# nantiferov/karpenter-sigs

Hardware: AMD Instinct MI355X
Metric: pods/sec in Scheduler.Solve @50k pods x 400 types (higher is better)
Workload: dtype int64; 1 GPU; C2: 50000 resource-only pods x 400 fake.InstanceTypes, 1 NodeClaimTemplate, no limits, empty topology (BenchmarkScheduling shape); pods=50000, instance_types=400, parallelism=replicas1, new_nodeclaims=122

## Files before the change

### karpenter-sigs_amd/csrc/ks_capi.cpp

```cpp
#include <hip/hip_runtime_api.h>

#include <algorithm>
#include <chrono>
#include <cstring>
#include <memory>
#include <mutex>
#include <string>
#include <vector>

#include "../../include/karpenter_amd.h"
#include "ks_archive.h"
#include "ks_feas.h"
#include "ks_feas_host.h"
#include "ks_host.h"
#include "ks_runtime.h"
#include "ks_sort_probe.h"

using namespace ks;

static thread_local std::string g_err;
namespace ks {
void set_last_error(const std::string& m) { g_err = m; }

static thread_local std::vector<Route>* g_routes = nullptr;
// ... 1092 lines not shown
  long long nfail = 0, nshared = 0, nverr = 0;
  for (char x : h.injectFailed) nfail += x ? 1 : 0;
  for (int32_t f : h.tab.pod_flags) {
    nshared += (f & PF_VSHARED) ? 1 : 0;
    nverr += (f & PF_VOLERR) ? 1 : 0;
  }
  kv("volAny", d.volAny); kv("volDrivers", d.VD); kv("volPvcs", d.NVU); kv("volLogCap", d.vLogCap);
  kv("volSharedPods", nshared); kv("volErrorPods", nverr); kv("injectFailed", nfail);
  kv("volStaticMounts", (long long)(h.tab.pod_vsbeg.empty() ? 0 : h.tab.pod_vsbeg.back()));
  o += "," + topo_inspect_json(h);
  std::vector<int32_t> frontBeg, frontPos;
  pareto_fronts(d, h.tab.tpl_it_beg, h.tab.tpl_its, h.tab.it_alloc, frontBeg, frontPos);
  o += ",\"runFuse\":" + std::to_string(run_fuse_build()) + ",\"sortLeaf\":" + std::to_string(sort_leaf_build()) +
       ",\"closedShift\":" + std::to_string(closed_shift_build()) + ",\"tplMasks\":" + std::to_string(tpl_masks_build()) +
       ",\"logRuns\":" + std::to_string(log_runs_build()) + ",\"sortRegs\":" + std::to_string(sort_regs_build()) +
       ",\"sortRegsN64\":" + std::to_string(sort_regs_n64_build()) + ",\"queuePacked\":" + std::to_string(queue_packed_build()) + ",\"paretoFronts\":[";
  for (int t = 0; t < d.NTPL; t++) {
    o += t ? ",[" : "[";
    for (int i = frontBeg[(size_t)t]; i < frontBeg[(size_t)t + 1]; i++)
      o += (i > frontBeg[(size_t)t] ? "," : "") + std::to_string(frontPos[(size_t)i]);
    o += "]";
  }
  o += "]";
  o += ",\"plans\":{";
  const size_t budgets[] = {160 * 1024 - 256, 6000, 9000, 14000, 24000, 40000};
  long long fnr = 0;
  for (int32_t f : h.tab.st_flags) fnr += (f & SF_HAS_KEYS) ? 1 : 0;
  KsDims pd = d;
  pd.fnOn = node_rows_on(d, (size_t)fnr);
  auto plan_json = [&](size_t budget, int wide) {
    Plan pl = make_plan(pd, budget, false, wide, (int)frontPos.size());
// ... 377 lines not shown
    ksjson::quote(o, r->errors[i].second);
  }
  o += "},\"stats\":{";
  static const char* names[] = {"nclaims", "ncommits", "hostnameCounter", "error", "pops", "algBytes",
                                "sorts", "sortsWithDescent", "claimFull", "claimQuickFail", "windows",
                                "cycPop", "cycNodes", "cycSort", "cycQuick", "cycFull", "cycCommit", "cycTemplates",
                                "cycTotal", "cycNodeCommit", "cycFullRs", "cycFullThr", "cycFullMasks", "cycFullApply",
                                "runs", "runPods", "sortsExact", "fineTopoPop", "fineState", "fineRefill",
                                "fineWindowTests", "fineWindowBlocks", "fineRecord", "fineNodeCommit", "fineWindowTopo",
                                "runCross", "runCrossStops", "runCrossLost", "sortsClosed", "tplMemoHits",
                                "cycSortFast", "cycSortExact", "cycSortClosed", "sortsLe12", "sortsLt50",
                                "cycRunCap", "cycCross", "cycBulk", "cycLog", "cycTplDerive", "cycTplStore",
                                "cycTplMax", "runCapFront", "runCapFull", "runCrossClosed", "runMoves",
                                "cycSortExactLe12", "cycSortExactLt50", "cycSortExactGe50", "closedShiftDiff",
                                "tplMaskFills", "tplMaskHits", "runRecs", "sortsRegs", "sortRegsBail", "sortRegsOver",
                                "cycTplCand", "cycTplFeas", "cycTplFilter", "cycTplThr", "cycLogLoad", "cycLogStore"};
  static_assert(sizeof(names) / sizeof(names[0]) == CT_NCOUNTERS, "one name per counter");
  for (int i = 0; i < CT_NCOUNTERS; i++) o += std::string(i ? "," : "") + "\"" + names[i] + "\":" + std::to_string(r->counters[i]);
  if (!r->routes.empty()) {
    std::string last = routes_json({r->routes.back()});
    o += ",\"route\":" + last.substr(1, last.size() - 3) + ",\"launches\":" + routes_json(r->routes) + "}";
  }
  o += ",\"plan\":{\"wide\":" + std::to_string(r->planWide) + ",\"KO\":" + std::to_string(r->plan.KO) +
       ",\"KL\":" + std::to_string(r->plan.KL) + ",\"talloc\":" + std::to_string(r->plan.talloc) +
       ",\"lds\":" + std::to_string(r->plan.lds) + "}";
  o += "}}";
  *json_out = strdup(o.c_str());
  return KS_OK;
  API_CATCH
}

// ... 304 lines not shown
```

### karpenter-sigs_amd/csrc/ks_problem.h

```cpp
#pragma once
#include <stdint.h>

#include "ks_reqset.h"

#if defined(__HIP_DEVICE_COMPILE__)
#define KS_G __attribute__((address_space(1)))
#define KS_L __attribute__((address_space(3)))
#define KS_C __attribute__((address_space(4)))
#else
#define KS_G
#define KS_L
#define KS_C
#endif

namespace ks {

constexpr int kMaxR = 16;
constexpr int kProbeMaxN = 1024;
constexpr int kMaxTpl = 64;
constexpr int kWave = 64;

enum PodStatus : int32_t { ST_PENDING = 0, ST_SCHEDULED = 1, ST_FAILED = 2 };
enum FailCode : uint32_t {
  FC_NONE = 0,
// ... 255 lines not shown
  CT_STEP,
  CT_RUN_CAP_FRONT = CT_STEP + 12,
  CT_RUN_CAP_FULL,
  CT_RUN_CROSS_CLOSED,
  CT_RUN_MOVES,
  CT_CYC_EXACT_BY_N,
  CT_CLOSED_SHIFT_DIFF = CT_CYC_EXACT_BY_N + 3,
  CT_TPL_MASK_FILLS,
  CT_TPL_MASK_HITS,
  CT_RUN_RECS,
  CT_SORT_REGS,
  CT_SORT_REGS_BAIL,
  CT_SORT_REGS_OVER,
  CT_CYC_SPLIT,
  CT_CYC_SPLIT_END = CT_CYC_SPLIT + 6,
  CT_NCOUNTERS = CT_CYC_SPLIT_END
};
enum SplitSub { YS_TPL_CAND = 0, YS_TPL_FEAS, YS_TPL_FILTER, YS_TPL_THR, YS_LOG_LOAD, YS_LOG_STORE };

enum StepSub {
  SS_SORT_FAST = 0,
  SS_SORT_EXACT,
  SS_SORT_CLOSED,
  SS_SORTS_LE12,
  SS_SORTS_LT50,
  SS_RUN_CAP,
  SS_CROSS,
  SS_BULK,
  SS_LOG,
  SS_TPL_DERIVE,
  SS_TPL_STORE,
  SS_TPL_MAX,
};
// ... 4 lines not shown
```

### karpenter-sigs_amd/csrc/ks_queue.hip

```cpp
#include <hip/hip_runtime.h>

#ifndef KS_QUEUE_PACKED
#define KS_QUEUE_PACKED 0
#endif

#include <hipcub/hipcub.hpp>

#include "ks_problem.h"

namespace ks {

__global__ void k_qkeys(const int64_t* sortkey, int comp, int64_t minv, const int32_t* perm, uint64_t* keys,
                        int32_t* vals, int n, int first) {
  const int i = blockIdx.x * blockDim.x + threadIdx.x;
  if (i >= n) return;
  const int p = first ? i : perm[i];
  keys[i] = (uint64_t)(sortkey[(int64_t)p * 4 + comp] - minv);
  vals[i] = p;
}

struct QPack {
  int64_t minv[4];
  int32_t shift[4];
  int32_t bits[4];
// ... 216 lines not shown
```

### karpenter-sigs_amd/csrc/ks_runtime.h

```cpp
#pragma once
#include <atomic>
#include <hip/hip_runtime_api.h>

#include <string>
#include <vector>

#include "../../include/karpenter_amd.h"
#include "ks_host.h"
#include "ks_tplmask.h"

namespace ks {
hipError_t launch_solve(const KsDev& D, const KsWork* works_dev, int nrep, const Plan& pl, int32_t* qorder,
                        uint64_t* skeys, int32_t* svals, void* stemp, size_t stempBytes, hipStream_t st,
                        hipEvent_t mid, const int32_t* fixed_order = nullptr, hipEvent_t* feas = nullptr,
                        int32_t* run_len = nullptr, uint64_t* run_words = nullptr, hipEvent_t post = nullptr);
hipError_t launch_sims(const KsDev& D, const KsWork* works_dev, int nsims, const Plan& pl, hipStream_t st);
hipError_t launch_sims_topo(const KsDev& D, const KsWork* w, int n, const Plan& pl, hipStream_t st);
void launch_feasibility(const KsDev& D, hipStream_t st);
void launch_feasibility_nodes(const KsDev& D, hipStream_t st);
bool sims_mw_supported(const KsDev& D, const Plan& pl);
hipError_t launch_sims_split(const KsDev& D, const KsWork* works_dev, int nsims, int nmw, const Plan& pl, hipStream_t st,
                             hipStream_t st2, hipEvent_t fork, hipEvent_t join);
int run_fuse_build();
int sort_leaf_build();
int closed_shift_build();
int tpl_masks_build();
int log_runs_build();
int sort_regs_build();
int sort_regs_n64_build();
int queue_packed_build();
hipError_t claim_sort_probe(int32_t* keys, int32_t* order, int n, int mode, int pos, int R, const int32_t* ctpl,
                            const int64_t* chead, int32_t* ptpl, int64_t* phead, int32_t* how, hipStream_t st);
Plan make_plan(const KsDims& d, size_t budget, bool sim = false, int wideKO = 0, int frontTotal = 0);
size_t queue_sort_temp_bytes(int n);
hipError_t queue_sort(const KsDev& D, uint64_t* keys, int32_t* vals, void* temp, size_t tempBytes, int32_t* out,
                      hipStream_t st);
hipError_t rank_from_order(const int32_t* order, int32_t* rank, int n, hipStream_t st);
hipError_t rec_headers(const int32_t* recs, int ns, int recWords, int TW, const int32_t* tplBeg, int ntpl, int32_t* hdr,
                       unsigned long long* status, unsigned* counter, unsigned long long* statusOut, hipStream_t st);
hipError_t sim_run_lengths(const int32_t* podmap, const int32_t* entry_sim, const int64_t* pod_req, const uint64_t* pod_s0,
                           const int32_t* pod_flags, int R, int n, uint64_t* words, int32_t* run_len, hipStream_t st,
                           bool strict = false);
hipError_t sim_queue_sort(const int32_t* rank, const int32_t* entries, const int32_t* entry_sim, int n, int rbits,
                          int sbits, uint64_t* keys, int32_t* vals, void* temp, size_t tempBytes, int32_t* out,
                          hipStream_t st);
// ... 108 lines not shown
```

### karpenter-sigs_amd/csrc/ks_solve.hip

```cpp
#include <hip/hip_runtime.h>

#ifndef KS_FM_OFF
#define KS_FM_OFF 0
#endif
#ifndef KS_TU
#define KS_TU 0
#endif
#ifndef KS_RUN_MIN
#define KS_RUN_MIN 3
#endif
#ifndef KS_NODE_K
#define KS_NODE_K 2
#endif
#ifndef KS_SORT_LANE0
#define KS_SORT_LANE0 0
#endif
#ifndef KS_SORT_LEAF
#define KS_SORT_LEAF 1
#endif
#ifndef KS_CLAIM_RUNS
#define KS_CLAIM_RUNS 1
#endif
#ifndef KS_RUN_CROSS
#define KS_RUN_CROSS 1
// ... 19 lines not shown
#ifndef KS_SORT_REGS_N64
#define KS_SORT_REGS_N64 1
#endif
#ifndef KS_TPL_MEMO
#define KS_TPL_MEMO 1
#endif
#ifndef KS_LOG_AHEAD
#define KS_LOG_AHEAD 0
#endif
#ifndef KS_TPL_MASKS
#define KS_TPL_MASKS 0
#endif
#ifndef KS_LOG_RUNS
#define KS_LOG_RUNS 1
#endif

#include "ks_gosort.h"
#include "ks_problem.h"
#include "ks_reqset.h"
#include "ks_sort_regs.h"
#include "ks_tplmask.h"

namespace ks {

using LI32 = int32_t KS_L*;
using LI64 = int64_t KS_L*;
using LU32 = uint32_t KS_L*;
using LU64 = uint64_t KS_L*;
using GI32 = int32_t KS_G*;
using GI64 = int64_t KS_G*;
// ... 918 lines not shown
  LU32 s_firr;
  enum : int { MM_T = 0, MM_CNT, MM_FOK, MM_POD = 4 };
  static constexpr bool TPL_MEMO = KS_TPL_MEMO && LEAN && !SIM;
  LU32 s_memo;
  int64_t memoHits = 0;
  static constexpr bool TPL_MASKS = KS_TPL_MASKS && LEAN && !SIM;
  LU32 s_tmask;
  LU32 s_tmv;
  int64_t maskFills = 0, maskHits = 0;
  static constexpr bool RUN_FRONT = KS_RUN_FRONT && KS_CLAIM_RUNS && LEAN && !SIM;
  enum : int { TPL_FOK = 1 << 30 };
  static __device__ __forceinline__ int tplv(int x) { return RUN_FRONT ? x & ~(int)TPL_FOK : x; }
  LI32 s_fbeg;
  LI32 s_front;
  mutable int64_t capFront = 0, capFull = 0;
  LU32 s_rmv;
  LU32 s_tch;
  LU32 s_tchr;
  LU32 s_tvol;
  LI32 s_tgm;
  LI32 s_tmin;
  LU32 s_trs0;
  LU32 s_trs1;
  LI32 s_tdom;
  LI32 s_tdw;
  LI32 s_live;
  LI32 s_tcs;
  LU32 s_tcd;
  LU64 s_gw;
  uint64_t t_mask = 0;
// ... 5 lines not shown
  uint64_t t_rss = 0;
  const uint32_t KS_G* fnp = nullptr;
  bool t_nonode = false;
  uint64_t t_active = ~0ull;
  int64_t algbytes = 0;
  bool rem_same = false;
  uint64_t cur_hpc = 0, cur_hpu = 0;
  uint64_t cur_hpo = 0;
  enum : int { VO_DB = 0, VO_DE, VO_SB, VO_SE, VO_NSP, VO_UB, VO_UE, VO_NLOG, VO_NSLOT, VO_WORDS };
  LI32 s_vol;
#ifdef KS_PHASE_STATS
  mutable uint64_t scyc[4] = {0, 0, 0, 0};
  mutable uint64_t xcyc[12] = {0, 0, 0, 0, 0, 0, 0, 0, 0, 0, 0, 0};
  uint64_t ecyc[3] = {0, 0, 0};
  mutable uint64_t ycyc[6] = {0, 0, 0, 0, 0, 0};
#endif

  __device__ Solver(const KsDev& D_, const KsWork KS_C& W_, const Plan& p_) : D(D_), d(D_.d), W(W_), pl(p_) {}
  __device__ __forceinline__ int R() const { return RT > 0 ? RT : d.R; }

  template <bool INL>
  __device__ __forceinline__ const ClaimView<INL>& cv() const {
    if constexpr (INL) return lc;
    else return gc;
  }

  template <class P>
  __device__ __forceinline__ bool fits(const int64_t* req, P alloc) const {
    bool ok = true;
#pragma unroll
// ... 840 lines not shown
#pragma unroll
      for (int r = 0; r < RM; r++) {
        if (RT == 0 && r >= d.R) break;
        nxt[r] = nthr[r] < nIT ? tsort_a((int64_t)tb * R() + (int64_t)r * nIT + nthr[r]) : INT64_MAX;
        moves |= nxt[r] < req[r];
      }
      if (!changed && !moves) {
        algbytes += 16 * R() + 4 * R();
        PHS_END(u1, 1);
        rem_same = true;
        ncnt = uni(v.cnt[c]);
        return ncnt > 0;
      }
      copy_words(s_rem, v.rem + (int64_t)c * d.TW, d.TW);
      wsync();
      for (int r = 0; r < R(); r++) {
        const int64_t base = (int64_t)tb * R() + (int64_t)r * nIT;
        int k = nthr[r];
        if (!(nxt[r] < req[r])) continue;
        while (k < nIT) {
          const int i = k + lane();
          const bool ex = i < nIT && tsort_a(base + i) < req[r];
          const uint64_t m = wballot(ex);
          if (m == 0) break;
          bool was = false;
          if (ex) {
            const int pos = tsort_p(base + i);
            const uint32_t bit = 1u << (pos & 31);
            was = (lds_and(s_rem + (pos >> 5), ~bit) & bit) != 0;
          }
          removed += __popcll(wballot(was));
          const int nm = __popcll(m);
          k += nm;
          examined += nm;
          if (nm < kWave) break;
        }
        nthr[r] = k;
      }
      algbytes += 8 * d.TW + 16 * R() + 4 * R() + (int64_t)examined * 12;
      wsync();
      PHS_END(u1, 1);
      if (!changed) {
        ncnt = uni(v.cnt[c]) - removed;
        return ncnt > 0;
      }
      PH_BEGIN(u2);
      feas_masks(s_rs, t, fm_row(s, t));
      PHS_END(u2, 2);
      PH_BEGIN(u3);
      for (int w0 = 0; w0 < d.TW; w0 += kWave) {
        const int w = w0 + lane();
        uint32_t keep = 0, irr = 0;
        if (w < d.TW) {
          const uint32_t rem = s_rem[w];
          irr = rem & s_firr[w];
// ... 96 lines not shown
    const ClaimView<INL>& v = cv<INL>();
    const int okNew = uni(s_okey[pos]) + 1;
    const bool srt = pos + 1 >= n || okNew <= uni(s_okey[pos + 1]);
    int64_t heads[RM];
#pragma unroll
    for (int r = 0; r < RM; r++) {
      if (RT == 0 && r >= d.R) break;
      heads[r] = s_phead[(int64_t)pos * R() + r];
    }
#pragma unroll
    for (int r = 0; r < RM; r++) {
      if (RT == 0 && r >= d.R) break;
      v.req[(int64_t)c * R() + r] = req[r];
      v.thr[(int64_t)c * R() + r] = nthr[r];
      s_phead[(int64_t)pos * R() + r] = heads[r] - pod[r];
    }
    v.cnt[c] = ncnt;
    s_okey[pos] = okNew;
    if (hpA()) W.c_hp[c] |= cur_hpu;
    if (keys(sflags) || (TOPO && t_any)) copy_words(W.c_rs + (int64_t)c * d.RSW, s_rs, d.RSW);
    if (!rem_same) copy_words(v.rem + (int64_t)c * d.TW, s_rem, d.TW);
    log_commit(p, c, nlog);
    if (keys(sflags) || !INL || hpA()) hbm_release();
    wsync();
    if (TOPO && t_rec) {
      if (keys(sflags) || t_any) topo_record(s_rs, c, -1, d.allowWK, nlog - 1);
      else topo_record(W.c_rs + (int64_t)c * d.RSW, c, -1, d.allowWK, nlog - 1);
    }
    algbytes += 24 * R() + 4 * d.TW + 8;
    return srt;
// ... 982 lines not shown
  }
  pl.KO = (int)ko;
  pl.KL = (int)kl;
  pl.lds = fixed + tclB + tdlB + livB + 3 * r16(4 * ko) + r16(8 * ko * R) + 2 * r16(4 * kl) + 2 * r16(8 * kl * R) + r16(4 * kl * TW) +
           r16(4 * kl * R) + (pl.tsort ? tsortB : 0) + (pl.talloc ? tallocB : 0) + (pl.tmask ? tmaskB : 0);
  return pl;
}

int run_fuse_build() { return KS_RUN_FUSE; }
int tpl_masks_build() { return KS_TPL_MASKS; }
int log_runs_build() { return KS_LOG_RUNS && KS_CLAIM_RUNS; }
int sort_leaf_build() { return KS_SORT_LEAF && !KS_SORT_LANE0; }
int closed_shift_build() { return KS_CLOSED_SHIFT && KS_SORT_CLOSED; }
int sort_regs_build() { return KS_SORT_REGS != 0 && KS_SORT_OUTLINE; }
int sort_regs_n64_build() { return sort_regs_build() && KS_SORT_REGS_N64; }

template <int R>
__global__ __attribute__((amdgpu_flat_work_group_size(64, 64))) void k_claim_sort_probe(
    int32_t* keys, int32_t* order, int n, int mode, int pos, const int32_t* ctpl, const int64_t* chead, int32_t* ptpl,
    int64_t* phead, int32_t* how) {
  extern __shared__ __attribute__((aligned(16))) char smem_probe[];
  char KS_L* sp = (char KS_L*)smem_probe;
  const size_t n4 = (4 * (size_t)n + 15) & ~(size_t)15;
  ClaimSort cs;
  LI64 s_phead = (LI64)sp;
  cs.s_okey = (LI32)(sp + 8 * (size_t)n * R);
  cs.s_order = (LI32)(sp + 8 * (size_t)n * R + n4);
  LI32 s_ptpl = (LI32)(sp + 8 * (size_t)n * R + 2 * n4);
  auto gather = [&](int lo, int hi) {
    for (int j = lo + lane(); j <= hi; j += kWave) {
// ... 151 lines not shown
```

### karpenter-sigs_amd/csrc/ks_solve_body.inc

```
  constexpr int RM = Solver<RT, TL, SIM, TOPO, LEAN>::RM;
#ifdef KS_FORCE_UNIFORM
  constexpr bool FORCEU = SIM || !LEAN;
#else
  constexpr bool FORCEU = SIM && LEAN;
#endif
  auto U = [](bool x) { return FORCEU ? ub(x) : x; };
  auto UI = [](int x) { return FORCEU ? uni(x) : x; };
  KS_BODY_SMEM_DECL
  const KsWork KS_C& W = KS_BODY_WORK;
  const KsDims& d = D.d;
  Solver<RT, TL, SIM, TOPO, LEAN> S(D, W, pl);
  const int R = S.R();
  char KS_L* sp = smem;
  auto take = [&](size_t bytes) { char KS_L* r = sp; sp += (bytes + 15) & ~(size_t)15; return r; };
  KeyMeta KS_L* s_keys = (KeyMeta KS_L*)take(sizeof(KeyMeta) * d.NK);
  S.s_order = (LI32)take(4 * (size_t)pl.KO);
  S.s_okey = (LI32)take(4 * (size_t)pl.KO);
  S.s_ptpl = (LI32)take(4 * (size_t)pl.KO);
  S.s_phead = (LI64)take(8 * (size_t)pl.KO * R);
  S.lc.tpl = (LI32)take(4 * (size_t)pl.KL);
  S.lc.req = (LI64)take(8 * (size_t)pl.KL * R);
  S.lc.max = (LI64)take(8 * (size_t)pl.KL * R);
  S.lc.rem = (LU32)take(4 * (size_t)pl.KL * d.TW);
  S.lc.thr = (LI32)take(4 * (size_t)pl.KL * R);
// ... 8 lines not shown
  S.s_rem = (LU32)take(4 * (size_t)d.TW + 8);
  S.s_cand = (LU32)take(4 * (size_t)d.TW + 8);
  S.s_fic = (LU32)take(4 * (size_t)d.TW + 8);
  S.s_fof = (LU32)take(4 * (size_t)d.TW + 8);
  S.s_firr = (LU32)take(4 * (size_t)d.TW + 8);
  constexpr bool MEMO = Solver<RT, TL, SIM, TOPO, LEAN>::TPL_MEMO;
  S.s_memo = (LU32)take(MEMO ? 4 * (size_t)tpl_memo_words(R, d.TW) : 0);
  if constexpr (MEMO) S.s_memo[S.MM_T] = (uint32_t)-1;
  constexpr bool MASKS = Solver<RT, TL, SIM, TOPO, LEAN>::TPL_MASKS;
  S.s_tmask = (LU32)take(MASKS && pl.tmask ? 4 * (size_t)tpl_mask_words(d.NTPL, d.TW) : 0);
  S.s_tmv = (LU32)take(MASKS && pl.tmask ? 4 * (size_t)d.NTPL : 0);
  if constexpr (MASKS) {
    if (pl.tmask)
      for (int i = lane(); i < d.NTPL; i += kWave) S.s_tmv[i] = 0;
  }
  constexpr bool FRONT = Solver<RT, TL, SIM, TOPO, LEAN>::RUN_FRONT;
  S.s_fbeg = (LI32)take(FRONT ? 4 * (size_t)(d.NTPL + 1) : 0);
  S.s_front = (LI32)take(FRONT ? 4 * (size_t)D.frontTotal : 0);
  const int NWN = (d.N + 31) >> 5;
  S.s_rmv = (LU32)take(SIM ? 4 * (size_t)NWN : 0);
  S.s_tch = (LU32)take(SIM ? 4 * (size_t)NWN : 0);
  S.s_tchr = (LU32)take(SIM || d.fnOn ? 4 * (size_t)NWN : 0);
  S.s_tvol = (LU32)take(SIM ? 4 * (size_t)NWN : 0);
  S.s_vol = (LI32)take(!LEAN && d.volAny ? 4 * (size_t)Solver<RT, TL, SIM, TOPO, LEAN>::VO_WORDS : 0);
  if (!LEAN && d.volAny)
    for (int i = lane(); i < Solver<RT, TL, SIM, TOPO, LEAN>::VO_WORDS; i += kWave) S.s_vol[i] = 0;
  S.s_tgm = (LI32)take(4 * (size_t)d.G * TGM_WORDS);
  S.s_tmin = (LI32)take(4 * (size_t)d.G);
  S.s_trs0 = (LU32)take(d.G ? 4 * (size_t)d.RSW : 0);
  S.s_trs1 = (LU32)take(d.G ? 4 * (size_t)d.RSW : 0);
// ... 188 lines not shown
  constexpr bool SORTC = Solver<RT, TL, SIM, TOPO, LEAN>::SORT_CLOSED;
  int dpos = -1;
  int64_t sortsClosed = 0;
  bool pushed = false;
  bool ident = !(SIM && W.sstart);
  bool anyRelaxed = false;
  uint32_t epoch = 1;
  int qhead = 0, qlen = P;
  if (SIM && !ident) S.sim_queue_init(P);
  int wn = 0, wi = 0;
  int64_t pops = 0, sorts = 0, slow = 0, exact = 0, windows = 0, fulls = 0, fullFails = 0, runs = 0, runPods = 0;
  int64_t cross = 0, crossStops = 0, crossLost = 0;
  int64_t crossClosed = 0, runMoves = 0;
  int stopC = -1;
  int64_t sortB = 0, pendSortB = 0;
  const int64_t popCap = (int64_t)64 * (d.S + P) + 100000;
  int err = KE_OK;
  Window<RT> w;
  int64_t pod[RM];
  int64_t req[RM];
  int nthr[RM];
  constexpr bool RSK = TOPO && !SIM;
  int rskip = 0;
  int64_t prqv = 0;
  constexpr bool LIVE = !SIM && !LEAN && NW > 0;
  const bool liveOn = LIVE && pl.livl > 0;
#ifndef KS_LIVE_ALL
#define KS_LIVE_ALL 1
#endif
  const bool liveAll = KS_LIVE_ALL && liveOn && d.N > NW * kWave;
// ... 183 lines not shown
    const int p = rdl(w.p, wi);
    const int g = SIM ? rdl(w.g, wi) : p;
    const int uid = rdl(w.uid, wi);
    uint64_t ll = (uint64_t)rdl64((int64_t)w.ll, wi);
    if (S.dupU()) {
      hbm_release();
      ll = uni64((int64_t)ld_sc1(W.last_len + uid));
    }
    if (U((uint32_t)(ll >> 32) == epoch && (uint32_t)ll == (uint32_t)qlen)) break;
    qhead = qhead + 1 == P ? 0 : qhead + 1;
    qlen--;
    if (++pops > popCap) { err = KE_ITER_CAP; break; }
    const int64_t abPop = S.algbytes;
    const int prevStop = stopC;
    stopC = -1;
    const int s = rdl(w.s, wi);
    const int sflags = rdl(w.flags, wi);
    const uint64_t toltpl = (uint64_t)rdl64((int64_t)w.toltpl, wi);
    const uint64_t tol0 = (uint64_t)rdl64((int64_t)w.tol0, wi), tol1 = (uint64_t)rdl64((int64_t)w.tol1, wi);
    if (S.hpA()) {
      S.cur_hpc = (uint64_t)rdl64((int64_t)w.hpc, wi);
      S.cur_hpu = (uint64_t)rdl64((int64_t)w.hpu, wi);
      S.cur_hpo = (uint64_t)rdl64((int64_t)w.hpo, wi);
    }
    const int pfl = S.volA() ? rdl(w.pf, wi) : 0;
    if (S.volA()) S.vol_pop(g, pfl);
    PH_BEGIN(tst);
    if (S.keys(sflags)) {
      S.copy_words(S.s_pin, D.st_rs + (int64_t)s * d.RSW, d.RSW);
      S.fnp = d.fnOn ? D.st_fn + (int64_t)uni(D.st_fnrow[s]) * ((d.N + 31) >> 5) : nullptr;
// ... 14 lines not shown
    wi++;
    if (RSK || liveOn) {
      int64_t mine = 0;
#pragma unroll
      for (int r = 0; r < RM; r++) {
        if (RT == 0 && r >= R) break;
        mine = lane() == r ? pod[r] : mine;
      }
      const bool differ = wballot(lane() < R && mine != prqv) != 0;
      if (RSK) rskip = differ || d.tgUnlab || d.negReq ? 0 : rskip;
      liveOK = liveOK && !differ;
      prqv = mine;
    }
    PH_END(t0, 0);
    bool placed = false;
    int rfirst = -1;
    PH_BEGIN(t1);
    const bool skipNodes = (TOPO && S.t_nonode && !d.tgUnlab) || (S.volA() && (pfl & PF_VOLERR));
    int scanFrom = 0;
    if constexpr (NW > 0) {
      if (d.N > 0 && !skipNodes && !(TOPO && d.tgUnlab) && !liveAll) {
        int kj = -1;
        uint64_t mj = 0;
        asm volatile("; KS_MARK window_begin");
        PH_BEGIN(twin);
        if constexpr (MWK) kj = mw_fit(pod, tol0, tol1, mj);
#pragma unroll
        for (int k = 0; k < (MWK ? 0 : NW); k++) {
          if (RSK && (k + 1) * kWave <= rskip) continue;
          const int n = k * kWave + lane();
          bool rok = true;
          if constexpr (FREEW) {
#pragma unroll
// ... 208 lines not shown
          S.node_store_rs(j, nrs);
          if (S.t_rec) S.topo_record(S.s_rs, -1, -1, 0, nlog);
        } else if (TOPO && S.t_rec) {
          S.topo_record(S.node_rs(j), -1, j, 0, nlog);
        }
        S.log_commit(p, -(j + 1), nlog);
        PH_END(t7, 7);
        placed = true;
      } else if (!useLive) {
        S.algbytes += (int64_t)min(KN * kWave, d.N - base) * (16 * R + 16);
      }
    }
    if (useLive && !placed) S.algbytes += (int64_t)(d.N - scanFrom) * (16 * R + 16);
    SPHS_END(S, tls, 3);
    PH_END(t1, 1);
    if (RSK && !skipNodes && d.N > 0) rskip = rfirst >= 0 ? rfirst : useLive ? scanFrom : d.N;
    const bool simNoClaim = SIM && TOPO && S.t_nonode && d.NTPL > 0;
    if (U(!placed && nclaims > 0)) {
      PH_BEGIN(t2);
      sorts++;
      sortB = pendSortB;
      S.algbytes += pendSortB;
      pendSortB = 0;
      if (!U(srt)) {
        const int64_t ab = S.algbytes;
        int npos;
        const int how = S.sort_claims(nclaims, SORTC ? dpos : -1, npos);
        exact += how == S.SORT_EXACT;
        sortsClosed += how == S.SORT_CLOSED_FORM;
        slow++;
// ... 14 lines not shown
          const int jj = base + ctz64(m);
          m &= m - 1;
          const int c = uni(S.s_order[jj]);
          PH_BEGIN(t4);
          const bool inl = c < pl.KL;
          int ncnt = 0;
          const bool ok = U(inl ? S.template claim_full<true>(c, s, sflags, pod, req, nthr, ncnt)
                                 : S.template claim_full<false>(c, s, sflags, pod, req, nthr, ncnt));
          fulls++;
          PH_END(t4, 4);
          PH_BEGIN(t5);
          if (ok) {
            srt = U(inl ? S.template commit_claim<true>(c, jj, nclaims, p, sflags, pod, req, nthr, ncnt, nlog)
                         : S.template commit_claim<false>(c, jj, nclaims, p, sflags, pod, req, nthr, ncnt, nlog));
            placed = true;
            if constexpr (SORTC) dpos = srt ? -1 : jj;
            if constexpr (LEAN && !SIM && KS_CLAIM_RUNS) {
              if (KS_RUN_CROSS && prevStop == c) crossLost++;
              if ((srt || KS_RUN_CROSS) && (ident || wi < wn)) {
                int m;
                if (ident) {
                  m = rdl(w.rl, wi - 1) - 1;
                  m = m < qlen ? m : qlen;
                } else {
                  bool inrun = false;
                  if (lane() >= wi && lane() < wn) {
                    bool same = w.toltpl == toltpl && w.tol0 == tol0 && w.tol1 == tol1;
#pragma unroll
                    for (int r = 0; r < RM; r++) {
                      if (RT == 0 && r >= R) break;
                      same &= w.req[r] == pod[r];
                    }
                    const uint32_t qx = (uint32_t)(qlen - (lane() - wi));
                    inrun = same && !((uint32_t)(w.ll >> 32) == epoch && (uint32_t)w.ll == qx);
                  }
                  const uint64_t nr = wballot(!inrun) & (~0ull << wi);
                  m = (nr ? ctz64(nr) : kWave) - wi;
                }
                m = UI(m);
                if (m > 0) {
                  int pos = jj, k;
                  int64_t credit;
                  const int64_t ab0 = S.algbytes;
                  if constexpr (KS_RUN_CROSS) {
                    PH_BEGIN(trc);
                    const int cap = inl ? S.template claim_run_cap<true>(c, pod, m) : S.template claim_run_cap<false>(c, pod, m);
                    SXPH_END(S, trc, SS_RUN_CAP);
                    PH_BEGIN(tcl);
                    int left = m < cap ? m : cap, K = uni(S.s_okey[jj]);
                    const int64_t qbytes = 8 * R + 4;
                    const int64_t span0 = ab0 - abPop - sortB - (int64_t)min((jj / kWave + 1) * kWave, nclaims) * qbytes;
                    int64_t per = ab0 - abPop;
                    k = 0;
                    credit = 0;
                    if constexpr (KS_RUN_FUSE && SORTC) {
                      int pos0 = jj, p = jj;
                      while (U(left > 0)) {
                        if (!srt) {
                          int hint = 0;
                          if (nclaims >= 50) (void)S.w_choose_pivot_moved(nclaims, pos0, p, K, hint);
                          if (hint == 1) {
// ... 163 lines not shown
                      seg = seg < left ? seg : left;
                      if (seg <= 0) break;
                      K += seg;
                      left -= seg;
                      k += seg;
                      credit += (int64_t)seg * per;
                      srt = K <= nx;
                      S.s_okey[pos] = K;
                      wsync();
                    }
                    SXPH_END(S, tcl, SS_CROSS);
                  } else {
                    const int cj = uni(S.s_okey[jj]);
                    const int nx = jj + 1 < nclaims ? uni(S.s_okey[jj + 1]) : 0x3fffffff;
                    const int M = m < nx - cj + 1 ? m : nx - cj + 1;
                    k = inl ? S.template claim_run_cap<true>(c, pod, M) : S.template claim_run_cap<false>(c, pod, M);
                    credit = (int64_t)k * (ab0 - abPop);
                  }
                  if (k > 0) {
                    int64_t podk[RM];
#pragma unroll
                    for (int r = 0; r < RM; r++) podk[r] = (int64_t)k * pod[r];
                    int kcnt = 0;
                    PH_BEGIN(tbk);
                    if (inl) (void)S.template claim_full<true>(c, s, sflags, podk, req, nthr, kcnt);
                    else (void)S.template claim_full<false>(c, s, sflags, podk, req, nthr, kcnt);
                    const int kk = KS_RUN_CROSS ? 0 : k;
                    srt = inl ? S.template commit_bulk<true>(c, pos, nclaims, kk, podk, req, nthr, kcnt)
                              : S.template commit_bulk<false>(c, pos, nclaims, kk, podk, req, nthr, kcnt);
                    if constexpr (SORTC) dpos = srt ? -1 : pos;
                    S.algbytes = ab0 + credit;
// ... 31 lines not shown
                        SYPH_END(S, tyq, YS_LOG_LOAD);
                        PH_BEGIN(tyb);
                        S.log_batch(k - b < kWave ? k - b : kWave, pv, c, nlog);
                        SYPH_END(S, tyb, YS_LOG_STORE);
                      }
                    }
                    SXPH_END(S, tlg, SS_LOG);
                    qhead += k;
                    if (qhead >= P) qhead -= P;
                    qlen -= k;
                    pops += k;
                    wi += k;
                    if (wi > wn) wi = wn;
                    runs++;
                    runPods += k;
                  }
                }
              }
            }
          } else {
            fullFails++;
            stepFF++;
            const int t = inl ? S.tplv(uni(S.lc.tpl[c])) : uni(W.c_tpl[c]);
            if (inl) S.template recompute_max<true>(c, S.lc.rem + (int64_t)c * d.TW, t, jj);
            else S.template recompute_max<false>(c, S.gc.rem + (int64_t)c * d.TW, t, jj);
          }
          PH_END(t5, 5);
        }
      }
    }
    if (!U(placed)) {
      PH_BEGIN(t6);
      const int r = U(simNoClaim) ? S.sim_template_calls(hostCtr)
                                  : UI(S.try_templates(p, s, sflags, toltpl, pod, nclaims, nlog, hostCtr, srt));
      PH_END(t6, 6);
      nclaims = UI(nclaims);
      hostCtr = UI(hostCtr);
      srt = U(srt);
      dpos = -1;
      if (r < 0) { err = KE_CLAIM_CAP; break; }
      if (r == 1) placed = true;
      if (r == 2) {
        W.pod_status[p] = ST_SCHEDULED;
        placed = true;
      }
    }
    if (U(placed)) {
      if (SIM && rdl(w.st, wi - 1) == ST_FAILED) W.pod_status[p] = ST_SCHEDULED;
      continue;
    }
    if constexpr (LEAN && !SIM) {
      if (d.dupUids) {
        err = KE_LEAN_EXIT;
        break;
      }
    }
    if (SIM && ident) S.sim_queue_init(P);
    const int s0 = D.pod_state0[g], ns = D.pod_nstate[g];
    const bool relaxed = U(s - s0 + 1 < ns);
    W.pod_status[p] = ST_FAILED;
    W.pod_fstate[p] = s;
    if (relaxed) W.pod_state[p] = s + 1;
// ... 46 lines not shown
    W.counters[CT_RUN_CROSS_LOST] = crossLost;
    W.counters[CT_SORT_CLOSED] = sortsClosed;
    W.counters[CT_TPL_MEMO_HITS] = S.memoHits;
    W.counters[CT_RUN_CAP_FRONT] = S.capFront;
    W.counters[CT_RUN_CAP_FULL] = S.capFull;
    W.counters[CT_RUN_CROSS_CLOSED] = crossClosed;
    W.counters[CT_RUN_MOVES] = runMoves;
    W.counters[CT_TPL_MASK_FILLS] = S.maskFills;
    W.counters[CT_TPL_MASK_HITS] = S.maskHits;
    W.counters[CT_RUN_RECS] = S.runRecs;
    if constexpr (decltype(S)::SORT_REGS) {
      W.counters[CT_SORT_REGS] = S.sortsRegs;
      W.counters[CT_SORT_REGS_BAIL] = S.sortRegsBail;
      W.counters[CT_SORT_REGS_OVER] = S.sortRegsOver;
    }
#ifdef KS_PHASE_STATS
    for (int i = 0; i < 7; i++) W.counters[CT_CYC_POP + i] = (int64_t)cyc[i];
    W.counters[CT_CYC_TOTAL] = (int64_t)(__builtin_amdgcn_s_memtime() - tstart);
    W.counters[CT_CYC_NCOMMIT] = (int64_t)cyc[7];
    for (int i = 0; i < 4; i++) W.counters[CT_CYC_SUB + i] = (int64_t)S.scyc[i];
    for (int i = 0; i < 8; i++) W.counters[CT_FINE + i] = (int64_t)fcyc[i];
    for (int i = 0; i < 12; i++) W.counters[CT_STEP + i] = (int64_t)S.xcyc[i];
    for (int i = 0; i < 3; i++) W.counters[CT_CYC_EXACT_BY_N + i] = (int64_t)S.ecyc[i];
    W.counters[CT_CLOSED_SHIFT_DIFF] = S.shiftDiff;
    for (int i = 0; i < 6; i++) W.counters[CT_CYC_SPLIT + i] = (int64_t)S.ycyc[i];
#endif
  }
  if constexpr (SIM) S.sim_record(P, nclaims, hostCtr, allSched, err, !ident, anyRelaxed);
```

Measured before the change: 8.075 million pods/s.

## Add capacity-bound run-cap skip, enable packed queue, add thr-batch and run-chain options

After a claim commit, the new code records whether the pod's request exceeds the remaining headroom in any resource. When it does, the next claim_run_cap call is skipped, since no further identical pod can fit. The packed queue layout is switched on by default. Batched threshold scanning and run chaining, which skips the node scan for consecutive identical pods, are added behind flags that default to off, together with new counters and per-kind cycle stats. The risk is that an over-conservative skip shortens runs or changes how placement proceeds.

```diff
diff --git a/karpenter-sigs_amd/csrc/ks_capi.cpp b/karpenter-sigs_amd/csrc/ks_capi.cpp
--- a/karpenter-sigs_amd/csrc/ks_capi.cpp
+++ b/karpenter-sigs_amd/csrc/ks_capi.cpp
@@ -1130,7 +1130,9 @@
   o += ",\"runFuse\":" + std::to_string(run_fuse_build()) + ",\"sortLeaf\":" + std::to_string(sort_leaf_build()) +
        ",\"closedShift\":" + std::to_string(closed_shift_build()) + ",\"tplMasks\":" + std::to_string(tpl_masks_build()) +
        ",\"logRuns\":" + std::to_string(log_runs_build()) + ",\"sortRegs\":" + std::to_string(sort_regs_build()) +
-       ",\"sortRegsN64\":" + std::to_string(sort_regs_n64_build()) + ",\"queuePacked\":" + std::to_string(queue_packed_build()) + ",\"paretoFronts\":[";
+       ",\"sortRegsN64\":" + std::to_string(sort_regs_n64_build()) + ",\"queuePacked\":" + std::to_string(queue_packed_build()) +
+       ",\"capBound\":" + std::to_string(cap_bound_build()) + ",\"thrBatch\":" + std::to_string(thr_batch_build()) +
+       ",\"runChain\":" + std::to_string(run_chain_build()) + ",\"paretoFronts\":[";
   for (int t = 0; t < d.NTPL; t++) {
     o += t ? ",[" : "[";
     for (int i = frontBeg[(size_t)t]; i < frontBeg[(size_t)t + 1]; i++)
@@ -1538,7 +1540,10 @@
                                 "cycTplMax", "runCapFront", "runCapFull", "runCrossClosed", "runMoves",
                                 "cycSortExactLe12", "cycSortExactLt50", "cycSortExactGe50", "closedShiftDiff",
                                 "tplMaskFills", "tplMaskHits", "runRecs", "sortsRegs", "sortRegsBail", "sortRegsOver",
-                                "cycTplCand", "cycTplFeas", "cycTplFilter", "cycTplThr", "cycLogLoad", "cycLogStore"};
+                                "cycTplCand", "cycTplFeas", "cycTplFilter", "cycTplThr", "cycLogLoad", "cycLogStore",
+                                "capBoundSkips", "thrBatchCalls", "thrMultiChunk", "chainPods",
+                                "cycStepOpen", "cycStepRun", "cycStepSingle", "stepsOpen", "stepsRun", "stepsSingle",
+                                "thrMoves", "cycThrMove", "runCapZero"};
   static_assert(sizeof(names) / sizeof(names[0]) == CT_NCOUNTERS, "one name per counter");
   for (int i = 0; i < CT_NCOUNTERS; i++) o += std::string(i ? "," : "") + "\"" + names[i] + "\":" + std::to_string(r->counters[i]);
   if (!r->routes.empty()) {
diff --git a/karpenter-sigs_amd/csrc/ks_problem.h b/karpenter-sigs_amd/csrc/ks_problem.h
--- a/karpenter-sigs_amd/csrc/ks_problem.h
+++ b/karpenter-sigs_amd/csrc/ks_problem.h
@@ -293,9 +293,16 @@
   CT_SORT_REGS_OVER,
   CT_CYC_SPLIT,
   CT_CYC_SPLIT_END = CT_CYC_SPLIT + 6,
-  CT_NCOUNTERS = CT_CYC_SPLIT_END
+  CT_CAP_BOUND_SKIPS = CT_CYC_SPLIT_END,
+  CT_THR_BATCH_CALLS,
+  CT_THR_MULTI_CHUNK,
+  CT_CHAIN_PODS,
+  CT_KIND,
+  CT_KIND_END = CT_KIND + 9,
+  CT_NCOUNTERS = CT_KIND_END
 };
 enum SplitSub { YS_TPL_CAND = 0, YS_TPL_FEAS, YS_TPL_FILTER, YS_TPL_THR, YS_LOG_LOAD, YS_LOG_STORE };
+enum KindSub { KD_CYC_OPEN = 0, KD_CYC_RUN, KD_CYC_SINGLE, KD_N_OPEN, KD_N_RUN, KD_N_SINGLE, KD_THR_MOVES, KD_CYC_THR_MOVE, KD_CAP_ZERO };
 
 enum StepSub {
   SS_SORT_FAST = 0,
diff --git a/karpenter-sigs_amd/csrc/ks_queue.hip b/karpenter-sigs_amd/csrc/ks_queue.hip
--- a/karpenter-sigs_amd/csrc/ks_queue.hip
+++ b/karpenter-sigs_amd/csrc/ks_queue.hip
@@ -1,7 +1,7 @@
 #include <hip/hip_runtime.h>
 
 #ifndef KS_QUEUE_PACKED
-#define KS_QUEUE_PACKED 0
+#define KS_QUEUE_PACKED 1
 #endif
 
 #include <hipcub/hipcub.hpp>
diff --git a/karpenter-sigs_amd/csrc/ks_runtime.h b/karpenter-sigs_amd/csrc/ks_runtime.h
--- a/karpenter-sigs_amd/csrc/ks_runtime.h
+++ b/karpenter-sigs_amd/csrc/ks_runtime.h
@@ -29,6 +29,9 @@
 int sort_regs_build();
 int sort_regs_n64_build();
 int queue_packed_build();
+int cap_bound_build();
+int thr_batch_build();
+int run_chain_build();
 hipError_t claim_sort_probe(int32_t* keys, int32_t* order, int n, int mode, int pos, int R, const int32_t* ctpl,
                             const int64_t* chead, int32_t* ptpl, int64_t* phead, int32_t* how, hipStream_t st);
 Plan make_plan(const KsDims& d, size_t budget, bool sim = false, int wideKO = 0, int frontTotal = 0);
diff --git a/karpenter-sigs_amd/csrc/ks_solve.hip b/karpenter-sigs_amd/csrc/ks_solve.hip
--- a/karpenter-sigs_amd/csrc/ks_solve.hip
+++ b/karpenter-sigs_amd/csrc/ks_solve.hip
@@ -57,6 +57,15 @@
 #ifndef KS_LOG_RUNS
 #define KS_LOG_RUNS 1
 #endif
+#ifndef KS_CAP_BOUND
+#define KS_CAP_BOUND 1
+#endif
+#ifndef KS_THR_BATCH
+#define KS_THR_BATCH 0
+#endif
+#ifndef KS_RUN_CHAIN
+#define KS_RUN_CHAIN 0
+#endif
 
 #include "ks_gosort.h"
 #include "ks_problem.h"
@@ -1005,6 +1014,12 @@
   LI32 s_fbeg;
   LI32 s_front;
   mutable int64_t capFront = 0, capFull = 0;
+  static constexpr bool CAP_BOUND = KS_CAP_BOUND && KS_CLAIM_RUNS && LEAN && !SIM;
+  static constexpr bool RUN_CHAIN = KS_RUN_CHAIN && KS_CLAIM_RUNS && LEAN && !SIM;
+  bool capOver = false;
+  int64_t capBoundSkips = 0;
+  static constexpr bool THR_BATCH = KS_THR_BATCH && LEAN && !SIM;
+  int64_t thrBatchCalls = 0, thrMultiChunk = 0;
   LU32 s_rmv;
   LU32 s_tch;
   LU32 s_tchr;
@@ -1040,6 +1055,7 @@
   mutable uint64_t xcyc[12] = {0, 0, 0, 0, 0, 0, 0, 0, 0, 0, 0, 0};
   uint64_t ecyc[3] = {0, 0, 0};
   mutable uint64_t ycyc[6] = {0, 0, 0, 0, 0, 0};
+  mutable uint64_t kcyc[9] = {0, 0, 0, 0, 0, 0, 0, 0, 0};
 #endif
 
   __device__ Solver(const KsDev& D_, const KsWork KS_C& W_, const Plan& p_) : D(D_), d(D_.d), W(W_), pl(p_) {}
@@ -1910,10 +1926,46 @@
       }
       copy_words(s_rem, v.rem + (int64_t)c * d.TW, d.TW);
       wsync();
+#ifdef KS_PHASE_STATS
+      const uint64_t tmv = __builtin_amdgcn_s_memtime();
+      kcyc[KD_THR_MOVES] += moves;
+#endif
+      [[maybe_unused]] bool more[RM] = {};
+      if constexpr (THR_BATCH) {
+        int pos[RM];
+        bool ex[RM];
+        uint32_t old[RM];
+        thrBatchCalls++;
+#pragma unroll
+        for (int r = 0; r < RM; r++) {
+          if (RT == 0 && r >= d.R) break;
+          const int i = nthr[r] + lane(), ii = i < nIT ? i : (nIT > 0 ? nIT - 1 : 0);
+          const int64_t base = (int64_t)tb * R() + (int64_t)r * nIT;
+          ex[r] = (nxt[r] < req[r]) & (i < nIT) & (tsort_a(base + ii) < req[r]);
+          pos[r] = tsort_p(base + ii);
+        }
+#pragma unroll
+        for (int r = 0; r < RM; r++) {
+          if (RT == 0 && r >= d.R) break;
+          const int q = ex[r] ? pos[r] : 0;
+          old[r] = lds_and(s_rem + (q >> 5), ex[r] ? ~(1u << (q & 31)) : ~0u);
+        }
+#pragma unroll
+        for (int r = 0; r < RM; r++) {
+          if (RT == 0 && r >= d.R) break;
+          const bool was = ex[r] & (((old[r] >> (pos[r] & 31)) & 1u) != 0);
+          const int nm = __popcll(wballot(ex[r]));
+          removed += __popcll(wballot(was));
+          nthr[r] += nm;
+          examined += nm;
+          more[r] = nm == kWave;
+        }
+      }
+      bool multi = false;
       for (int r = 0; r < R(); r++) {
         const int64_t base = (int64_t)tb * R() + (int64_t)r * nIT;
         int k = nthr[r];
-        if (!(nxt[r] < req[r])) continue;
+        if (THR_BATCH ? !more[r] : !(nxt[r] < req[r])) continue;
         while (k < nIT) {
           const int i = k + lane();
           const bool ex = i < nIT && tsort_a(base + i) < req[r];
@@ -1931,10 +1983,15 @@
           examined += nm;
           if (nm < kWave) break;
         }
+        if constexpr (THR_BATCH) multi |= k > nthr[r];
         nthr[r] = k;
       }
+      if constexpr (THR_BATCH) thrMultiChunk += multi;
       algbytes += 8 * d.TW + 16 * R() + 4 * R() + (int64_t)examined * 12;
       wsync();
+#ifdef KS_PHASE_STATS
+      if (moves) kcyc[KD_CYC_THR_MOVE] += __builtin_amdgcn_s_memtime() - tmv;
+#endif
       PHS_END(u1, 1);
       if (!changed) {
         ncnt = uni(v.cnt[c]) - removed;
@@ -2061,6 +2118,15 @@
       v.req[(int64_t)c * R() + r] = req[r];
       v.thr[(int64_t)c * R() + r] = nthr[r];
       s_phead[(int64_t)pos * R() + r] = heads[r] - pod[r];
+    }
+    if constexpr (CAP_BOUND) {
+      bool over = false;
+#pragma unroll
+      for (int r = 0; r < RM; r++) {
+        if (RT == 0 && r >= d.R) break;
+        over |= pod[r] > heads[r] - pod[r];
+      }
+      capOver = ub(over);
     }
     v.cnt[c] = ncnt;
     s_okey[pos] = okNew;
@@ -3073,6 +3139,9 @@
 int closed_shift_build() { return KS_CLOSED_SHIFT && KS_SORT_CLOSED; }
 int sort_regs_build() { return KS_SORT_REGS != 0 && KS_SORT_OUTLINE; }
 int sort_regs_n64_build() { return sort_regs_build() && KS_SORT_REGS_N64; }
+int cap_bound_build() { return KS_CAP_BOUND && KS_CLAIM_RUNS; }
+int thr_batch_build() { return KS_THR_BATCH; }
+int run_chain_build() { return KS_RUN_CHAIN && KS_CLAIM_RUNS; }
 
 template <int R>
 __global__ __attribute__((amdgpu_flat_work_group_size(64, 64))) void k_claim_sort_probe(
diff --git a/karpenter-sigs_amd/csrc/ks_solve_body.inc b/karpenter-sigs_amd/csrc/ks_solve_body.inc
--- a/karpenter-sigs_amd/csrc/ks_solve_body.inc
+++ b/karpenter-sigs_amd/csrc/ks_solve_body.inc
@@ -46,6 +46,8 @@
     if (pl.tmask)
       for (int i = lane(); i < d.NTPL; i += kWave) S.s_tmv[i] = 0;
   }
+  constexpr bool CAPB = Solver<RT, TL, SIM, TOPO, LEAN>::CAP_BOUND;
+  constexpr bool CHAINB = Solver<RT, TL, SIM, TOPO, LEAN>::RUN_CHAIN;
   constexpr bool FRONT = Solver<RT, TL, SIM, TOPO, LEAN>::RUN_FRONT;
   S.s_fbeg = (LI32)take(FRONT ? 4 * (size_t)(d.NTPL + 1) : 0);
   S.s_front = (LI32)take(FRONT ? 4 * (size_t)D.frontTotal : 0);
@@ -264,6 +266,8 @@
   int64_t crossClosed = 0, runMoves = 0;
   int stopC = -1;
   int64_t sortB = 0, pendSortB = 0;
+  bool chain = false;
+  int64_t nodeAB = 0, chainPods = 0;
   const int64_t popCap = (int64_t)64 * (d.S + P) + 100000;
   int err = KE_OK;
   Window<RT> w;
@@ -477,6 +481,12 @@
     const int64_t abPop = S.algbytes;
     const int prevStop = stopC;
     stopC = -1;
+    const bool chained = CHAINB && chain;
+    const int rlp = CHAINB ? rdl(w.rl, wi) : 0;
+    if constexpr (CHAINB) {
+      chain = false;
+      chainPods += chained;
+    }
     const int s = rdl(w.s, wi);
     const int sflags = rdl(w.flags, wi);
     const uint64_t toltpl = (uint64_t)rdl64((int64_t)w.toltpl, wi);
@@ -521,9 +531,15 @@
     }
     PH_END(t0, 0);
     bool placed = false;
+    bool onClaim = false;
+    int kRun = 0;
+#ifdef KS_PHASE_STATS
+    int skind = KD_CYC_SINGLE;
+#endif
     int rfirst = -1;
     PH_BEGIN(t1);
-    const bool skipNodes = (TOPO && S.t_nonode && !d.tgUnlab) || (S.volA() && (pfl & PF_VOLERR));
+    const bool skipNodes = (TOPO && S.t_nonode && !d.tgUnlab) || (S.volA() && (pfl & PF_VOLERR)) || chained;
+    const int64_t abNode = CHAINB ? S.algbytes : 0;
     int scanFrom = 0;
     if constexpr (NW > 0) {
       if (d.N > 0 && !skipNodes && !(TOPO && d.tgUnlab) && !liveAll) {
@@ -762,6 +778,10 @@
     if (useLive && !placed) S.algbytes += (int64_t)(d.N - scanFrom) * (16 * R + 16);
     SPHS_END(S, tls, 3);
     PH_END(t1, 1);
+    if constexpr (CHAINB) {
+      if (chained) S.algbytes += nodeAB;
+      else if (!placed) nodeAB = S.algbytes - abNode;
+    }
     if (RSK && !skipNodes && d.N > 0) rskip = rfirst >= 0 ? rfirst : useLive ? scanFrom : d.N;
     const bool simNoClaim = SIM && TOPO && S.t_nonode && d.NTPL > 0;
     if (U(!placed && nclaims > 0)) {
@@ -806,6 +826,7 @@
             srt = U(inl ? S.template commit_claim<true>(c, jj, nclaims, p, sflags, pod, req, nthr, ncnt, nlog)
                          : S.template commit_claim<false>(c, jj, nclaims, p, sflags, pod, req, nthr, ncnt, nlog));
             placed = true;
+            if constexpr (CHAINB) onClaim = true;
             if constexpr (SORTC) dpos = srt ? -1 : jj;
             if constexpr (LEAN && !SIM && KS_CLAIM_RUNS) {
               if (KS_RUN_CROSS && prevStop == c) crossLost++;
@@ -836,7 +857,15 @@
                   const int64_t ab0 = S.algbytes;
                   if constexpr (KS_RUN_CROSS) {
                     PH_BEGIN(trc);
-                    const int cap = inl ? S.template claim_run_cap<true>(c, pod, m) : S.template claim_run_cap<false>(c, pod, m);
+                    int cap = 0;
+                    if (CAPB && S.capOver) {
+                      S.capBoundSkips++;
+                    } else {
+                      cap = inl ? S.template claim_run_cap<true>(c, pod, m) : S.template claim_run_cap<false>(c, pod, m);
+#ifdef KS_PHASE_STATS
+                      S.kcyc[KD_CAP_ZERO] += cap == 0;
+#endif
+                    }
                     SXPH_END(S, trc, SS_RUN_CAP);
                     PH_BEGIN(tcl);
                     int left = m < cap ? m : cap, K = uni(S.s_okey[jj]);
@@ -1030,7 +1059,15 @@
                     const int cj = uni(S.s_okey[jj]);
                     const int nx = jj + 1 < nclaims ? uni(S.s_okey[jj + 1]) : 0x3fffffff;
                     const int M = m < nx - cj + 1 ? m : nx - cj + 1;
-                    k = inl ? S.template claim_run_cap<true>(c, pod, M) : S.template claim_run_cap<false>(c, pod, M);
+                    k = 0;
+                    if (CAPB && S.capOver) {
+                      S.capBoundSkips++;
+                    } else {
+                      k = inl ? S.template claim_run_cap<true>(c, pod, M) : S.template claim_run_cap<false>(c, pod, M);
+#ifdef KS_PHASE_STATS
+                      S.kcyc[KD_CAP_ZERO] += k == 0;
+#endif
+                    }
                     credit = (int64_t)k * (ab0 - abPop);
                   }
                   if (k > 0) {
@@ -1092,6 +1129,10 @@
                     if (wi > wn) wi = wn;
                     runs++;
                     runPods += k;
+                    if constexpr (CHAINB) kRun = k;
+#ifdef KS_PHASE_STATS
+                    skind = KD_CYC_RUN;
+#endif
                   }
                 }
               }
@@ -1118,12 +1159,38 @@
       dpos = -1;
       if (r < 0) { err = KE_CLAIM_CAP; break; }
       if (r == 1) placed = true;
+      if constexpr (CHAINB) onClaim = r == 1;
+#ifdef KS_PHASE_STATS
+      if (r == 1) skind = KD_CYC_OPEN;
+#endif
       if (r == 2) {
         W.pod_status[p] = ST_SCHEDULED;
         placed = true;
       }
     }
     if (U(placed)) {
+      if constexpr (CHAINB) {
+        if (onClaim && qlen > 0) {
+          bool nx = false;
+          if (ident) {
+            nx = rlp - 1 - kRun > 0;
+          } else if (wi < wn) {
+            bool same = lane() == wi && w.toltpl == toltpl && w.tol0 == tol0 && w.tol1 == tol1;
+#pragma unroll
+            for (int r = 0; r < RM; r++) {
+              if (RT == 0 && r >= R) break;
+              same &= w.req[r] == pod[r];
+            }
+            same &= !((uint32_t)(w.ll >> 32) == epoch && (uint32_t)w.ll == (uint32_t)qlen);
+            nx = wballot(same) != 0;
+          }
+          chain = nx;
+        }
+      }
+#ifdef KS_PHASE_STATS
+      S.kcyc[skind] += __builtin_amdgcn_s_memtime() - t0;
+      S.kcyc[skind + KD_N_OPEN] += 1;
+#endif
       if (SIM && rdl(w.st, wi - 1) == ST_FAILED) W.pod_status[p] = ST_SCHEDULED;
       continue;
     }
@@ -1200,6 +1267,12 @@
       W.counters[CT_SORT_REGS_BAIL] = S.sortRegsBail;
       W.counters[CT_SORT_REGS_OVER] = S.sortRegsOver;
     }
+    if constexpr (CAPB) W.counters[CT_CAP_BOUND_SKIPS] = S.capBoundSkips;
+    if constexpr (CHAINB) W.counters[CT_CHAIN_PODS] = chainPods;
+    if constexpr (decltype(S)::THR_BATCH) {
+      W.counters[CT_THR_BATCH_CALLS] = S.thrBatchCalls;
+      W.counters[CT_THR_MULTI_CHUNK] = S.thrMultiChunk;
+    }
 #ifdef KS_PHASE_STATS
     for (int i = 0; i < 7; i++) W.counters[CT_CYC_POP + i] = (int64_t)cyc[i];
     W.counters[CT_CYC_TOTAL] = (int64_t)(__builtin_amdgcn_s_memtime() - tstart);
@@ -1210,6 +1283,7 @@
     for (int i = 0; i < 3; i++) W.counters[CT_CYC_EXACT_BY_N + i] = (int64_t)S.ecyc[i];
     W.counters[CT_CLOSED_SHIFT_DIFF] = S.shiftDiff;
     for (int i = 0; i < 6; i++) W.counters[CT_CYC_SPLIT + i] = (int64_t)S.ycyc[i];
+    for (int i = 0; i < 9; i++) W.counters[CT_KIND + i] = (int64_t)S.kcyc[i];
 #endif
   }
   if constexpr (SIM) S.sim_record(P, nclaims, hostCtr, allSched, err, !ident, anyRelaxed);
```

Measured after the change: 8.631 million pods/s, median of 6. +6.9%, better.
